# AVianEco/Softspoken

Hardware: AMD Instinct MI355X
Metric: audio-seconds processed/sec (whole node), 16 kHz mono (higher is better)
Workload: dtype f16x2

## Files before the change

softspoken_amd/csrc/conv4.hip:

```cpp
#include "kernels.h"
#include <cstdio>
#include <cstdlib>
#include <type_traits>
#include <utility>

namespace ss {

#ifdef SS_DEVBUILD
static int dev_env(const char* name, int dflt) { const char* v = getenv(name); return v ? atoi(v) : dflt; }
#else
static constexpr int dev_env(const char*, int dflt) { return dflt; }
#endif

typedef float f32x16 __attribute__((ext_vector_type(16)));
typedef float f32x4 __attribute__((ext_vector_type(4)));
typedef float f32x2 __attribute__((ext_vector_type(2)));
typedef __bf16 bf16x8 __attribute__((ext_vector_type(8)));
typedef __bf16 bf16x2 __attribute__((ext_vector_type(2)));
typedef _Float16 f16x8 __attribute__((ext_vector_type(8)));
typedef _Float16 f16x2 __attribute__((ext_vector_type(2)));
typedef short s16x2 __attribute__((ext_vector_type(2)));
typedef uint32_t u32x4 __attribute__((ext_vector_type(4)));
typedef uint32_t u32x2 __attribute__((ext_vector_type(2)));

// ... 61 lines not shown
    constexpr int KC = 32;
    constexpr bool DUO = NH > 1;
    static_assert(!DUO || (NT == 1 && NW * NH == 16 && RP == 0 && !FIRST && !FLAT && !PF2), "DUO: the plain A / B launches");
    constexpr bool RING = DUO && !BRES;
    static_assert(!RING || (SPLIT && NH == 4), "RING: f16x2, four 4-wave tiles");
    static_assert(!SPLIT || !PF2, "SPLIT: single-stage prefetch");
    static_assert(!RANK1 || (SPLIT && !RES && !RADD), "RANK1: conv1_1.B in f16x2 mode");
    static_assert(!(FIRST && SPLIT) || RANK1, "FIRST in f16x2 mode: the block's residual is the fp32 rank-1 term");
    static_assert(!FLAT || (NT == 1 && NW == 8 && BRES && (RADD || RP) && !POOL && !FIRST), "FLAT: conv9_1.B");
    static_assert(!PF2 || (BRES && !FIRST), "two-stage prefetch: resident-weight launches");
    static_assert(RP == 0 || (!RES && !RADD && !FIRST), "RP: a B launch that computes the block's projection itself (no r tensor)");
    static_assert(!FIRST || (NT == 1 && BRES && !RES && !RADD), "FIRST: conv1_1.B, one 32 -> 32 chunk, rank-1 residual");
    constexpr int kTapBytes = 2 * NT * 1024;
    constexpr int TAPS = RES ? 10 : 9;
    constexpr int NTHR = 64 * NW;
    constexpr int TH = 2 * NW;
    constexpr int PR = TH + 2;
    constexpr int kA = PR * kRowPitch;
    constexpr int NPA = PR * kPatch * 4;
    constexpr int AIT = (NPA + NTHR - 1) / NTHR;
    constexpr int NPB = (SPLIT ? 2 : 1) * TAPS * kTapBytes / 16;
    constexpr int BIT = BRES ? 1 : (DUO ? (NPB / 2 + NTHR - 1) / NTHR : (NPB + NTHR - 1) / NTHR);
    static_assert(!(RES && (RADD || POOL)), "RES is the A launch; RADD / POOL belong to B launches");
    static_assert(AIT <= 4, "edge flags are packed 8 bits per piece");
    extern __shared__ __attribute__((aligned(16))) char smem[];

    const int half = DUO ? __builtin_amdgcn_readfirstlane((int)threadIdx.x / NTHR) : 0;
    const int tid = DUO ? (int)threadIdx.x % NTHR : (int)threadIdx.x, lane = tid & 63;
    const int wave = __builtin_amdgcn_readfirstlane(tid >> 6);
    const int hh = lane >> 5, m = lane & 31;
    const int py = (m >> 1) & 1, px = (m & 1) | ((m >> 2) << 1);
    char* sA = smem + half * kA;
    const int sb_bytes = RING ? 2 * lds_b_bytes : lds_b_bytes;
    char* sB = smem + NH * kA;
    const int proj_steps = RP ? (a.C0x + a.C1x) / 16 : 0;
    constexpr bool proj_lds = RP > 0 && (BRES || NT == 3 || SPLIT);
    const char* sProj = smem + NH * kA + sb_bytes;
    const int proj_tiles = SPLIT ? a.Cout / 32 : NT;
    const int proj_bank = proj_steps * proj_tiles * 1024;
    const float* sBias = (const float*)(sProj + (proj_lds ? (SPLIT ? 2 : 1) * proj_bank : 0));
    constexpr int FW = 20, FROWS = PR + 3;
    float* sFb = (float*)sBias + 32;
    float* sF = sFb + 32;
    float* sFlat = (float*)sBias + 32;

    const int H = a.H, W = a.W, Cout = a.Cout;
    const int ngroups = Cout / (32 * NT);
    const int nch_r = (a.C0 + a.C1) / KC;
    const int nch = SPLIT ? 2 * nch_r : nch_r;
    const int all_taps = nch_r * TAPS;

    const int xcd = blockIdx.x & 7, local = (int)(blockIdx.x >> 3) * NH + half, gper = (int)(gridDim.x >> 3) * NH;
    const int per = (total_tiles + 7) >> 3;
    auto tile_of = [&](int loc, int it) -> int {
        if constexpr (RING) {
            const int total_pos = total_tiles / ngroups, per_pos = (total_pos + 7) >> 3;
            const int idx = loc + (it / ngroups) * gper;
            const int pos = xcd * per_pos + idx;
            return (idx < per_pos && pos < total_pos) ? pos * ngroups + it % ngroups : -1;
        }
        const int idx = loc + it * gper;
        const int t = xcd * per + idx;
        return (idx < per && t < total_tiles) ? t : -1;
    };
    auto tile_at = [&](int it) -> int { return tile_of(local, it); };
    struct Tile { int n, y0, x0, g; };
    auto decode = [&](int t) -> Tile {
        Tile d;
        d.g = t % ngroups; t /= ngroups;
        d.x0 = (t % a.tiles_x) * 16; t /= a.tiles_x;
        d.y0 = (t % a.tiles_y) * TH;
        d.n = t / a.tiles_y;
        return d;
    };

    uint32_t pix_full[AIT], pix_half[AIT], lds_off[AIT], flags = 0;
    const uint32_t part16 = (tid & 3) * 16;
    {
        const int Wh = W >> 1;
#pragma unroll
        for (int it = 0; it < AIT; ++it) {
            const int p = tid + NTHR * it;
            const int pix = p >> 2;
            const int pyy = pix / kPatch, pxx = pix - pyy * kPatch;
            lds_off[it] = pyy * kRowPitch + pxx * kPixPitch + part16;
            pix_full[it] = pyy * W + pxx;
            pix_half[it] = ((pyy + 1) >> 1) * Wh + ((pxx + 1) >> 1);
            const uint32_t f = (pyy == 0 ? 1u : 0u) | (pyy == PR - 1 ? 2u : 0u) | (pxx == 0 ? 4u : 0u) | (pxx == kPatch - 1 ? 8u : 0u) |
                               (p >= NPA ? 16u : 0u);
            flags |= f << (8 * it);
        }
    }
    u32x4 ra0[AIT], ra1[AIT];
    u32x4 rb[BIT];
    float rf = 0.f;
    static_assert(!FIRST || (PR + 2) * FW <= NTHR, "one feature value per thread");

    auto issue_patch = [&](const Tile& d, int ci, u32x4 (&ra)[AIT]) {
        if constexpr (FIRST) {
            if constexpr (SPLIT) { if (ci & 1) return; }
            const int fy = tid / FW, fx = tid - fy * FW;
            const int Y = d.y0 - 2 + fy, X = d.x0 - 2 + fx;
            rf = (tid < (PR + 2) * FW && (unsigned)Y < (unsigned)H && (unsigned)X < (unsigned)W)
                     ? a.rank1_src[((size_t)d.n * H + Y) * W + X] : 0.f;
            return;
        }
        const int ch = (SPLIT ? ci >> 1 : ci) * KC;
        const int64_t plane = (SPLIT && !(ci & 1)) ? a.lo_delta : 0;
        const char* base; uint32_t cs2, toff; bool up;
        if (ch < a.C0) {
            base = (const char*)a.src0 - kHdr + plane; cs2 = 2u * a.C0; up = false;
            toff = kHdr + ((((uint32_t)d.n * H + d.y0 - 1) * W + d.x0 - 1) * a.C0 + ch) * 2u;
        } else {
            base = (const char*)a.src1 - kHdr + plane; cs2 = 2u * a.C1; up = true;
            toff = kHdr + ((((uint32_t)d.n * (H >> 1) + (d.y0 >> 1) - 1) * (W >> 1) + (d.x0 >> 1) - 1) * a.C1 + (ch - a.C0)) * 2u;
        }
        uint32_t tm = (d.y0 == 0 ? 1u : 0u) | (d.y0 + TH == H ? 2u : 0u) | (d.x0 == 0 ? 4u : 0u) | (d.x0 + 16 == W ? 8u : 0u) | 16u;
        const uint32_t tp = toff + part16;
#pragma unroll
        for (int it = 0; it < AIT; ++it) {
            const uint32_t pix = up ? pix_half[it] : pix_full[it];
            uint32_t off = __umul24(pix, cs2) + tp;
            if (flags & (tm << (8 * it))) off = 0;
            ra[it] = *(const u32x4*)(base + off);
        }
    };
    auto issue_weights = [&](const Tile& d, int ci) {
        if constexpr (!BRES && !RING) {
            if constexpr (SPLIT) { if (ci & 1) return; }
            const char* wsrc = SPLIT ? (const char*)a.wpk + ((size_t)d.g * nch_r + (ci >> 1)) * 2 * (TAPS * kTapBytes)
                                     : (const char*)a.wpk + ((size_t)d.g * all_taps + ci * TAPS) * kTapBytes;
#pragma unroll
            for (int it = 0; it < BIT; ++it) {
                const int p = tid + NTHR * it;
                u32x4 v = {0u, 0u, 0u, 0u};
                if (p < NPB) v = *(const u32x4*)(wsrc + p * 16);
                rb[it] = v;
            }
        }
    };
    auto commit = [&](u32x4 (&ra)[AIT], bool patch, bool bank) {
        if constexpr (FIRST) return;
        if (patch) {
#pragma unroll
            for (int it = 0; it < AIT; ++it) {
                if ((it + 1) * NTHR <= NPA || !(flags & (16u << (8 * it)))) *(u32x4*)(sA + lds_off[it]) = ra[it];
            }
        }
        if constexpr (!BRES && !RING) {
            if (bank) {
#pragma unroll
                for (int it = 0; it < BIT; ++it) {
                    const int p = tid + NTHR * it;
                    if (p < NPB) *(u32x4*)(sB + p * 16) = rb[it];
                }
            }
        }
    };
    constexpr int NPH = NPB / 2;
    auto ring_duty = [&](int s, int n_chunks) {
        if constexpr (RING) {
            if (half > 1) return;
            const int k = (s >> 1) + 1;
            if (k >= n_chunks) return;
            if (!(s & 1)) {
                const char* wsrc = (const char*)a.wpk + ((size_t)(k % (ngroups * nch_r)) * 2 + half) * (TAPS * kTapBytes);
#pragma unroll
                for (int it = 0; it < BIT; ++it) {
                    const int p = tid + NTHR * it;
                    u32x4 v = {0u, 0u, 0u, 0u};
                    if (p < NPH) v = *(const u32x4*)(wsrc + p * 16);
                    rb[it] = v;
                }
            } else {
                char* dst = sB + (k & 1) * lds_b_bytes + half * (TAPS * kTapBytes);
#pragma unroll
                for (int it = 0; it < BIT; ++it) {
                    const int p = tid + NTHR * it;
                    if (p < NPH) *(u32x4*)(dst + p * 16) = rb[it];
                }
            }
        }
    };

    constexpr int RPH = RP >= 2 ? RP / 2 : RP;
    u32x4 pxh[(SPLIT && RP) ? RPH : 1], pxl[(SPLIT && RP) ? RPH : 1];
    auto issue_proj = [&](const Tile& d, int chunk, auto k0c, auto k1c) {
        constexpr int K0 = decltype(k0c)::value, K1 = decltype(k1c)::value;
        if constexpr (SPLIT && RP > 0 && K1 > K0) {
            const uint32_t t_full = kHdr + ((((uint32_t)d.n * H + d.y0 + 2 * wave) * W + d.x0) * a.C0x) * 2u;
            const uint32_t t_half = kHdr + ((((uint32_t)d.n * (H >> 1) + (d.y0 >> 1) + wave) * (W >> 1) + (d.x0 >> 1)) * a.C1x) * 2u;
            uint32_t zl = 0;
            asm volatile("" : "+v"(zl));
            const uint32_t xf_o = (uint32_t)((py * W + px) * a.C0x + hh * 8) * 2u + zl, xh_o = (uint32_t)((px >> 1) * a.C1x + hh * 8) * 2u + zl;
#pragma unroll
            for (int k = K0; k < K1; ++k) {
                const int sidx = chunk * RP + k, ch = sidx * 16;
                const char* base; uint32_t off;
                if (sidx >= proj_steps) { base = (const char*)a.xp0 - kHdr; off = 0; }
                else if (ch < a.C0x) { base = (const char*)a.xp0 - kHdr; off = t_full + xf_o + ch * 2u; }
                else { base = (const char*)a.xp1 - kHdr; off = t_half + xh_o + (ch - a.C0x) * 2u; }
                pxh[k - K0] = *(const u32x4*)(base + off);
                pxl[k - K0] = *(const u32x4*)(base + a.lo_delta + off);
            }
        }
    };

    int it_tile = 0;
    struct Stage { int ci; Tile d; };
    auto next_stage = [&](const Stage& s0, Stage& n) -> bool {
        n = s0; n.ci = s0.ci + 1;
        if (n.ci == nch) {
            n.ci = 0;
            const int t = tile_at(++it_tile);
            if (t < 0) return false;
            n.d = decode(t);
        }
        return true;
    };
    int my_stages = 0, max_stages = 0;
    if constexpr (DUO) {
        const int l0 = (int)(blockIdx.x >> 3) * NH;
        int n0 = 0, nmine = 0;
        while (tile_of(l0, n0) >= 0) ++n0;
        while (tile_of(l0 + half, nmine) >= 0) ++nmine;
        my_stages = nmine * nch;
        max_stages = n0 * nch;
        if (max_stages == 0) return;
    } else {
        if (tile_at(0) < 0) return;
    }
    Stage cs{0, decode((DUO && my_stages == 0) ? 0 : tile_at(0))}, n1 = cs, n2 = cs;

    if constexpr (BRES || RING) {
        const char* wsrc = (const char*)a.wpk;
        for (int p = tid; p < lds_b_bytes / 16; p += NTHR) *(u32x4*)(sB + p * 16) = *(const u32x4*)(wsrc + (size_t)p * 16);
    }
    for (int i = tid; i < Cout * (RES ? 2 : 1); i += NTHR)
        ((float*)sBias)[i] = i < Cout ? a.bias[i] : a.res_bias[i - Cout];
    if constexpr (proj_lds)
        for (int p = tid; p < (SPLIT ? 2 : 1) * proj_steps * proj_tiles * 64; p += NTHR) *(u32x4*)((char*)sProj + p * 16) = *(const u32x4*)((const char*)a.proj_w + (size_t)p * 16);
    u32x4 wfirst = {0u, 0u, 0u, 0u}, wr1 = {0u, 0u, 0u, 0u}, wfirst_lo = {0u, 0u, 0u, 0u};
    constexpr int NMT = (PR * kPatch + 31) / 32;
    int pf_off[2], pa_off[2]; uint32_t pflags = 0;
    if constexpr (FIRST) {
        for (int i = tid; i < 32; i += NTHR) sFb[i] = a.first_b[i];
        for (int i = tid; i < FROWS * FW; i += NTHR) sF[i] = 0.f;
        const float* w9 = a.first_w;
        auto wv = [&](int t) { return w9[t * 32 + m]; };
        if constexpr (SPLIT) {
            auto hi2 = [&](float x, float y) { return pack_f16(x, y); };
            auto lo2 = [&](float x, float y) { const f32x2 b = unpack_f16(pack_f16(x, y)); return pack_f16(x - b[0], y - b[1]); };
            if (hh == 0) {
                wfirst = u32x4{hi2(wv(0), wv(1)), hi2(wv(2), 0.f), hi2(wv(3), wv(4)), hi2(wv(5), 0.f)};
                wfirst_lo = u32x4{lo2(wv(0), wv(1)), lo2(wv(2), 0.f), lo2(wv(3), wv(4)), lo2(wv(5), 0.f)};
            } else {
                wfirst = u32x4{hi2(wv(6), wv(7)), hi2(wv(8), 0.f), 0u, 0u};
                wfirst_lo = u32x4{lo2(wv(6), wv(7)), lo2(wv(8), 0.f), 0u, 0u};
            }
        } else if (hh == 0) {
            wfirst = u32x4{pack_bf16(wv(0), wv(1)), pack_bf16(wv(2), 0.f), pack_bf16(wv(3), wv(4)), pack_bf16(wv(5), 0.f)};
            const float w = a.rank1_w[m];
            const float whi = (float)(__bf16)w, wlo = w - whi;
            wr1 = u32x4{pack_bf16(whi, whi), pack_bf16(wlo, 0.f), 0u, 0u};
        } else {
            wfirst = u32x4{pack_bf16(wv(6), wv(7)), pack_bf16(wv(8), 0.f), 0u, 0u};
        }
#pragma unroll
        for (int t = 0; t < 2; ++t) {
            const int q = 32 * (wave + NW * t) + m;
            const bool in = q < PR * kPatch;
            const int qq = in ? q : 0;
            const int qy = qq / kPatch, qx = qq - qy * kPatch;
            pf_off[t] = (qy + 2 * hh) * FW + qx;
            pa_off[t] = qy * kRowPitch + qx * kPixPitch + hh * 16;
            const uint32_t f = (qy == 0 ? 1u : 0u) | (qy == PR - 1 ? 2u : 0u) | (qx == 0 ? 4u : 0u) | (qx == kPatch - 1 ? 8u : 0u) | (in ? 0u : 16u);
            pflags |= f << (8 * t);
        }
    }
    u32x4 hk_lo[(FIRST && SPLIT) ? 2 : 1], hk_hi[(FIRST && SPLIT) ? 2 : 1];
    auto produce = [&](const Tile& d, int part) {
        const uint32_t tm = (d.y0 == 0 ? 1u : 0u) | (d.y0 + TH == H ? 2u : 0u) | (d.x0 == 0 ? 4u : 0u) | (d.x0 + 16 == W ? 8u : 0u) | 16u;
#pragma unroll
        for (int t = 0; t < 2; ++t) {
            if (wave + NW * t < NMT) {
                if constexpr (SPLIT) {
                    if (part) {
                        if (!(pflags & (16u << (8 * t)))) {
// ... 889 lines not shown
```

softspoken_amd/csrc/conv4_ups.hip:

```cpp
#include "kernels.h"
#include <cstdlib>
#include <type_traits>

namespace ss {

namespace {

typedef float f32x16 __attribute__((ext_vector_type(16)));
typedef float f32x4 __attribute__((ext_vector_type(4)));
typedef float f32x2 __attribute__((ext_vector_type(2)));
typedef _Float16 f16x8 __attribute__((ext_vector_type(8)));
typedef _Float16 f16x2 __attribute__((ext_vector_type(2)));
typedef uint32_t u32x4 __attribute__((ext_vector_type(4)));
typedef uint32_t u32x2 __attribute__((ext_vector_type(2)));

constexpr int kHdr = 256;
constexpr int kPix = 80;
constexpr int kRowR = 1472;
constexpr int kOdd = 720;
constexpr int kRowU = 896;
constexpr int kLowPlane = 6 * kRowU;
constexpr int kPatchBytes = 10 * kRowR;
constexpr int kBankR = 9 * 2048, kBankU = 16 * 2048;
constexpr int NW = 4, NH = 4, NTHR = 64 * NW;
// ... 295 lines not shown
    for (int i = half; i < NH - 1; ++i) lds_barrier();
}

namespace {
constexpr int kEntR = 10 * 2048;
constexpr int kEntRH = kEntR + 256;
constexpr int kEntU = 17 * 2048;
constexpr int kSlot = kEntU;
constexpr int kGL = (kEntU / 32 + NTHR - 1) / NTHR;
}

__global__ __launch_bounds__(NTHR * NH) __attribute__((amdgpu_waves_per_eu(4)))
void conv3x3_upsr_kernel(ConvArgs a, int total_tiles, int) {
    extern __shared__ __attribute__((aligned(16))) char smem[];
#ifdef SS_DEVBUILD
#define SS_ABL(bit) (a.dbg & (1 << (bit)))
#else
#define SS_ABL(bit) false
#endif
    const int half = __builtin_amdgcn_readfirstlane((int)threadIdx.x / NTHR);
    const int tid = (int)threadIdx.x % NTHR, lane = tid & 63;
    const int wave = __builtin_amdgcn_readfirstlane(tid >> 6);
    const int hh = lane >> 5, m = lane & 31;
    const int ca = wave & 1, cb = wave >> 1;
    const int X = m & 7, Y = m >> 3;
    char* sA = smem + half * kPatchBytes;
    char* sR = smem + NH * kPatchBytes;

    const int H = a.H, W = a.W, Cout = a.Cout;
    const int ngroups = Cout / 32;
    const int nreg = a.C0 / 32, nups = a.C1 / 32;
    const int nst = 3 * nreg + 2 * nups;
    const int group_bytes = nreg * (kEntRH + kEntR) + nups * 2 * kEntU;

    struct Sp { int sec, chunk, part; };
    auto sp_next = [&](Sp& p) -> bool {
        if (++p.part == (p.sec ? 2 : 3)) {
            p.part = 0;
            if (++p.chunk == (p.sec ? nups : nreg)) {
                p.chunk = 0; p.sec ^= 1;
                if (p.sec && nups == 0) p.sec = 0;
                return p.sec == 0;
            }
        }
        return false;
    };
    auto starts_entry = [&](const Sp& p) -> bool { return p.sec || p.part != 1; };
    auto needs_patch = [&](const Sp& p) -> bool { return p.sec ? p.part == 0 : p.part != 2; };
    auto entry_off = [&](const Sp& p) -> int {
        return p.sec ? nreg * (kEntRH + kEntR) + (2 * p.chunk + p.part) * kEntU : p.chunk * (kEntRH + kEntR) + (p.part == 2 ? kEntRH : 0);
    };
    auto entry_size = [&](const Sp& p) -> int { return p.sec ? kEntU : (p.part == 2 ? kEntR : kEntRH); };

    const int xcd = blockIdx.x & 7, local = (int)(blockIdx.x >> 3) * NH + half, gper = (int)(gridDim.x >> 3) * NH;
    const int total_pos = total_tiles / ngroups, per_pos = (total_pos + 7) >> 3;
    const int lim = min(per_pos, total_pos - xcd * per_pos);
    auto count_pos = [&](int loc) -> int { return lim > loc ? (lim - loc + gper - 1) / gper : 0; };
    struct Tile { int n, y0, x0, g; };
    auto decode_pos = [&](int pos, int g) -> Tile {
        Tile d;
        d.g = g;
        d.x0 = (pos % a.tiles_x) * 16; pos /= a.tiles_x;
        d.y0 = (pos % a.tiles_y) * 8;
        d.n = pos / a.tiles_y;
        return d;
    };
    const int my_pos = count_pos(local);
    const int my_stages = my_pos * ngroups * nst;
    const int max_stages = count_pos((int)(blockIdx.x >> 3) * NH) * ngroups * nst;
    if (max_stages == 0) return;

    constexpr int AIT = 3;
    uint32_t pix_full[AIT], lds_off[AIT], flags = 0;
    const uint32_t part16 = (tid & 3) * 16;
#pragma unroll
    for (int it = 0; it < AIT; ++it) {
        const int p = tid + NTHR * it, pix = p >> 2;
        const int pyy = pix / 18, pxx = pix - pyy * 18;
        lds_off[it] = pyy * kRowR + (pxx & 1) * kOdd + (pxx >> 1) * kPix + part16;
        pix_full[it] = pyy * W + pxx;
        const uint32_t f = (pyy == 0 ? 1u : 0u) | (pyy == 9 ? 2u : 0u) | (pxx == 0 ? 4u : 0u) | (pxx == 17 ? 8u : 0u) | (p >= 720 ? 16u : 0u);
        flags |= f << (8 * it);
    }
    uint32_t pix_low, lds_low, flags_low;
    {
        const int pix = tid >> 2;
        const int ly = pix / 10, lx = pix - ly * 10;
        lds_low = ly * kRowU + lx * kPix + part16;
        pix_low = ly * (W >> 1) + lx;
        flags_low = (ly == 0 ? 1u : 0u) | (ly == 5 ? 2u : 0u) | (lx == 0 ? 4u : 0u) | (lx == 9 ? 8u : 0u) | (tid >= 240 ? 16u : 0u);
    }
    u32x4 ra[AIT];
    auto issue_patch = [&](const Tile& d, const Sp& p) {
        if (SS_ABL(18)) return;
        const uint32_t tm = (d.y0 == 0 ? 1u : 0u) | (d.y0 + 8 == H ? 2u : 0u) | (d.x0 == 0 ? 4u : 0u) | (d.x0 + 16 == W ? 8u : 0u) | 16u;
        if (p.sec == 0) {
            const int64_t plane = p.part ? 0 : a.lo_delta;
            const char* base = (const char*)a.src0 - kHdr + plane;
            const uint32_t cs2 = 2u * a.C0;
            const uint32_t tp = kHdr + ((((uint32_t)d.n * H + d.y0 - 1) * W + d.x0 - 1) * a.C0 + p.chunk * 32) * 2u + part16;
#pragma unroll
            for (int it = 0; it < AIT; ++it) {
                uint32_t off = __umul24(pix_full[it], cs2) + tp;
                if (flags & (tm << (8 * it))) off = 0;
                ra[it] = *(const u32x4*)(base + off);
            }
        } else {
            const char* base = (const char*)a.src1 - kHdr;
            const uint32_t cs2 = 2u * a.C1;
            const uint32_t tp = kHdr + ((((uint32_t)d.n * (H >> 1) + (d.y0 >> 1) - 1) * (W >> 1) + (d.x0 >> 1) - 1) * a.C1 + p.chunk * 32) * 2u + part16;
            uint32_t off = __umul24(pix_low, cs2) + tp;
            if (flags_low & tm) off = 0;
            ra[0] = *(const u32x4*)(base + off);
            ra[1] = *(const u32x4*)(base + (off ? a.lo_delta + off : 0));
        }
    };
    auto commit = [&](int sec) {
        if (sec == 0) {
#pragma unroll
            for (int it = 0; it < AIT; ++it)
                if (!(flags & (16u << (8 * it)))) *(u32x4*)(sA + lds_off[it]) = ra[it];
        } else if (!(flags_low & 16u)) {
            *(u32x4*)(sA + lds_low) = ra[0];
            *(u32x4*)(sA + kLowPlane + lds_low) = ra[1];
        }
    };

    const int pos0 = xcd * per_pos + local;
    Tile cur = decode_pos(my_pos ? pos0 : 0, 0), nxt = cur;
    int cur_g = 0, cur_j = 0, nxt_g = 0, nxt_j = 0;
    bool nxt_ok = false;
    auto compute_next = [&]() {
        nxt_g = cur_g + 1; nxt_j = cur_j;
        if (nxt_g == ngroups) { nxt_g = 0; ++nxt_j; }
        nxt_ok = nxt_j < my_pos;
        if (nxt_ok) nxt = decode_pos(pos0 + nxt_j * gper, nxt_g);
    };
    struct Cur { Sp sp; Tile d; bool ok; };
    auto advance = [&](Cur& c) {
        if (sp_next(c.sp)) { c.d = nxt; c.ok = nxt_ok; }
    };
    Cur ip{Sp{0, 0, 0}, cur, true};

    {
        Sp p{0, 0, 0};
        for (int e = 0; e < 3; ++e) {
            const char* src = (const char*)a.wpk + entry_off(p);
            const int np = entry_size(p) / 16;
            for (int q = (int)threadIdx.x; q < np; q += NTHR * NH) *(u32x4*)(sR + e * kSlot + q * 16) = *(const u32x4*)(src + (size_t)q * 16);
            do sp_next(p); while (!starts_entry(p));
        }
    }
    Sp rq{0, 0, 0};
    int rq_g = 0, rq_t = 0, rq_e = 0, rq_slot = 0;
    auto rq_advance = [&]() {
        if (starts_entry(rq)) { ++rq_e; rq_slot = rq_slot == 2 ? 0 : rq_slot + 1; }
        ++rq_t;
        if (sp_next(rq)) { if (++rq_g == ngroups) rq_g = 0; }
    };
    if (half & 1) for (int i = 0; i < (half == 1 ? 2 : 3); ++i) rq_advance();
    auto ring_issue = [&]() {
        if (!(half & 1)) return;
        if (!SS_ABL(19) && rq_t < max_stages && rq_e >= 3 && starts_entry(rq)) {
            const int total = entry_size(rq) / 16;
            const int h0 = ((total / 2 + 63) / 64) * 64;
            const int base = half == 1 ? 0 : h0, cnt = half == 1 ? h0 : total - h0;
            const char* src = (const char*)a.wpk + (size_t)rq_g * group_bytes + entry_off(rq) + base * 16;
            char* dst = sR + rq_slot * kSlot + base * 16 + wave * 1024;
#pragma unroll
            for (int it = 0; it < kGL; ++it) {
                const int idx = tid + NTHR * it;
                if (idx < cnt)
                    __builtin_amdgcn_global_load_lds((const __attribute__((address_space(1))) void*)(src + (size_t)idx * 16),
                                                     (__attribute__((address_space(3))) void*)(uintptr_t)(dst + it * NTHR * 16), 16, 0, 0);
            }
        }
        rq_advance();
    };

    issue_patch(ip.d, ip.sp);
    commit(0);
    if (my_stages == 0) ip.ok = false;
    else do advance(ip); while (ip.ok && !needs_patch(ip.sp));
    if (ip.ok) issue_patch(ip.d, ip.sp);
    __syncthreads();

    f32x16 acc, racc;
    auto mm = [&](const u32x4& w, const u32x4& x, const f32x16& c) -> f32x16 { return SS_ABL(16) ? c : mfma(w, x, c); };
    const int base_r = 2 * Y * kRowR + X * kPix + hh * 16;
    const int base_u = Y * kRowU + X * kPix + hh * 16;
    const int boff0 = lane * 16;
    const uint32_t st_off = (uint32_t)(((2 * Y + ca) * W + 2 * X + cb) * Cout + hh * 8) * 2u;
    const uint32_t r_lane = (uint32_t)(32 * hh + 4 * X + 2 * ca + cb) * 32u;
    int tap_r[9];
#pragma unroll
    for (int t = 0; t < 9; ++t) {
        const int dy = t / 3, dx = t % 3;
        tap_r[t] = (ca + dy) * kRowR + ((cb + dx) & 1) * kOdd + ((cb + dx) >> 1) * kPix;
    }
    int tap_u[4];
#pragma unroll
    for (int t = 0; t < 4; ++t) tap_u[t] = (ca + (t >> 1)) * kRowU + (cb + (t & 1)) * kPix;
    constexpr int kCentreU = kRowU + kPix;

    int jit_n = 0;
#ifdef SS_DEVBUILD
    uint32_t st_prev = 0, st_sub = 0, st_sum[9] = {0u, 0u, 0u, 0u, 0u, 0u, 0u, 0u, 0u};
#endif
    auto substamp = [&](int seg) {
#ifdef SS_DEVBUILD
        if (a.stamps) { const uint32_t t = (uint32_t)__builtin_amdgcn_s_memtime(); if (seg >= 5) st_sum[seg] += t - st_sub; st_sub = t; }
// ... 108 lines not shown
#pragma unroll
            for (int sub = 0; sub < 2; ++sub) {
                const u32x4 w = *(const u32x4*)(ent + boff0 + 16 * 2048 + sub * 1024);
                const u32x4 xh = *(const u32x4*)(sA + base_u + kCentreU + sub * 32), xl = *(const u32x4*)(sA + kLowPlane + base_u + kCentreU + sub * 32);
                racc = mm(w, xl, racc);
                racc = mm(w, xh, racc);
            }
        } else {
            const char* bb = ent + boff0 + wave * 4 * 2048;
            constexpr int PM = 3;
            u32x4 ph[PM], wf[PM];
            auto load2 = [&](int st, int slot) {
                if (SS_ABL(17)) return;
                const int tap = st >> 1, sub = st & 1;
                ph[slot] = *(const u32x4*)(sA + base_u + tap_u[tap] + sub * 32);
                wf[slot] = *(const u32x4*)(bb + tap * 2048 + sub * 1024);
            };
#pragma unroll
            for (int st = 0; st < PM - 1; ++st) load2(st, st);
#pragma unroll
            for (int st = 0; st < 8; ++st) {
                if (st + PM - 1 < 8) load2(st + PM - 1, (st + PM - 1) % PM);
                acc = mm(wf[st % PM], ph[st % PM], acc);
            }
#pragma unroll
            for (int sub = 0; sub < 2; ++sub) {
                const u32x4 w = *(const u32x4*)(ent + boff0 + 16 * 2048 + sub * 1024);
                const u32x4 xh = *(const u32x4*)(sA + base_u + kCentreU + sub * 32);
                racc = mm(w, xh, racc);
            }
        }
        if (a.dbg & 32) __builtin_amdgcn_s_setprio(0);
        jitter(1);
        vm_lds_barrier();
        jitter(2);
        const bool more = stage_no + 1 < my_stages;
        constexpr bool next_has_patch = KIND == 0 || KIND == 2 || KIND == 4;
        const int next_sec = KIND == 0 ? 0 : KIND == 2 ? ((c == nreg - 1 && nups) ? 1 : 0) : (c == nups - 1 ? 0 : 1);
        const bool np = next_has_patch && more;
        substamp(0);
        if (np) commit(next_sec);
        substamp(5);
        if (last && !SS_ABL(20)) {
            char* rq_p = (char*)a.res_out +
                         ((((((uint32_t)cur.n * (H >> 1) + (cur.y0 >> 1) + Y) * (W >> 4) + (cur.x0 >> 4)) * (uint32_t)ngroups) + cur.g) * 2048u + r_lane);
            *(f32x4*)(rq_p) = f32x4{racc[0], racc[1], racc[2], racc[3]};
            *(f32x4*)(rq_p + 16) = f32x4{racc[4], racc[5], racc[6], racc[7]};
            *(f32x4*)(rq_p + a.lo_delta) = f32x4{racc[8], racc[9], racc[10], racc[11]};
            *(f32x4*)(rq_p + a.lo_delta + 16) = f32x4{racc[12], racc[13], racc[14], racc[15]};
        }
        if (last) { acc_done = acc; done_off = (((uint32_t)cur.n * H + cur.y0) * W + cur.x0) * Cout + cur.g * 32; have_done = true; }
        if (KIND == 1 && c == 0 && have_done && !SS_ABL(20)) { store_h(); have_done = false; }
        if (KIND == 1 && c == 0) compute_next();
        if (last && more) { cur = nxt; cur_g = nxt_g; cur_j = nxt_j; }
        substamp(6);
        if (np) {
            do advance(ip); while (ip.ok && !needs_patch(ip.sp));
            if (ip.ok) issue_patch(ip.d, ip.sp);
        }
        substamp(7);
        ring_issue();
        substamp(8);
        jitter(3);
        lds_barrier();
        jitter(4);
        if (KIND != 0) e_slot = e_slot == 2 ? 0 : e_slot + 1;
        ++stage_no;
    };
    using K0 = std::integral_constant<int, 0>; using K1 = std::integral_constant<int, 1>; using K2 = std::integral_constant<int, 2>;
    using K3 = std::integral_constant<int, 3>; using K4 = std::integral_constant<int, 4>;
    const int my_pg = my_pos * ngroups, max_pg = max_stages / nst;
    for (int i = 0; i < half; ++i) lds_barrier();
    for (int pg = 0; pg < max_pg; ++pg) {
        if (pg < my_pg) {
            for (int c = 0; c < nreg; ++c) { stage(K0{}, c); stage(K1{}, c); stage(K2{}, c); }
            for (int c = 0; c < nups; ++c) { stage(K3{}, c); stage(K4{}, c); }
        } else {
            for (int st = 0; st < nst; ++st) { vm_lds_barrier(); ring_issue(); lds_barrier(); }
        }
    }
    for (int i = half; i < NH - 1; ++i) lds_barrier();
    if (have_done && !SS_ABL(20)) store_h();
#ifdef SS_DEVBUILD
    if (a.stamps && lane == 0) {
        uint32_t* sp = (uint32_t*)a.stamps + (((size_t)blockIdx.x * NH + half) * NW + wave) * 16;
        for (int i = 0; i < 5; ++i) sp[i] = st_sum[i];
        sp[5] = (uint32_t)jit_n; sp[6] = st_sum[5]; sp[7] = st_sum[6]; sp[8] = st_sum[7]; sp[9] = st_sum[8];
    }
#endif
#undef SS_ABL
}

namespace {

struct UpsChoice { bool ok; int total, lds_b, grid; size_t lds; };

UpsChoice choose_ups(ConvArgs& a, int num_cus) {
    UpsChoice c{};
    static const int on = dev_env("SOFTSPOKEN_UPS", 1);
    if (!on) return c;
    if (!a.plain || !a.src0 || !a.src1 || !a.out || !a.wpk || !a.bias || !a.range_flag || a.lo_delta <= 0) return c;
    if (a.res_out || a.res_in || a.pool_out || a.rank1_src || a.first_w || a.flat_part || a.proj_w || !a.relu || a.R0 || a.R1) return c;
    if (a.Cout != 32 || a.C0 < 32 || a.C1 < 32 || a.C0 % 32 || a.C1 % 32 || a.H % 8 || a.W % 16 || ((a.H | a.W) & 1)) return c;
    if ((double)a.N * a.H * a.W * std::max(a.Cout, std::max(a.C0, a.C1)) * 2.0 + kHdr >= 4294967296.0) return c;
    a.tiles_y = a.H / 8; a.tiles_x = a.W / 16;
    const long total_l = (long)a.N * a.tiles_y * a.tiles_x;
    if (total_l <= 0 || total_l > 0x7fffffff) return c;
    c.total = (int)total_l;
    c.lds_b = (a.C0 / 32) * 2 * kBankR + (a.C1 / 32) * 2 * kBankU;
    c.lds = (size_t)NH * kPatchBytes + c.lds_b + (size_t)a.Cout * 4;
    if (c.lds > 160 * 1024) return c;
    c.grid = (num_cus + 7) / 8 * 8;
    if (c.grid * NH > c.total) c.grid = ((c.total + NH - 1) / NH + 7) / 8 * 8;
    c.ok = true;
    return c;
}

}

namespace {

struct UpsrChoice { bool ok; int total, grid; size_t lds; };

UpsrChoice choose_upsr(ConvArgs& a, int num_cus) {
// ... 65 lines not shown
```

softspoken_amd/csrc/engine.hip:

```cpp
#include "engine.h"

#include <algorithm>
#include <chrono>
#include <cmath>
#include <cstdio>
#include <cstdlib>
#include <cstring>

namespace ss {

static thread_local std::string g_err;

int fail(ss_ctx* c, int code, const std::string& msg) {
    g_err = msg;
    if (c) c->err = msg;
    return code;
}
const char* thread_error() { return g_err.c_str(); }

#ifdef SS_DEVBUILD
int dev_env(const char* name, int dflt) { const char* v = getenv(name); return v ? atoi(v) : dflt; }
#endif

double now_ms() { return std::chrono::duration<double, std::milli>(std::chrono::steady_clock::now().time_since_epoch()).count(); }
// ... 71 lines not shown
    for (const WsTensor& t : kWsTensors) {
        offs.push_back(total + kActHeader);
        total += kActHeader + (((size_t)n * t.H * t.W * t.C * es + 255) & ~(size_t)255);
    }
    const int planes = c->prec == kF16x2 ? 2 : 1;
    const size_t feat_b = (size_t)n * 128 * 256 * 4, flat_b = (size_t)n * 64 * 4 * 256 * 4;
    hipError_t e = ws_malloc(c, &w.arena, total * planes);
    if (e != hipSuccess) { what = "activation workspace (" + std::to_string(total * planes >> 20) + " MiB)"; free_ws(w); return e; }
    if ((e = ws_malloc(c, (void**)&w.feat, feat_b)) != hipSuccess || (e = ws_malloc(c, (void**)&w.flat, flat_b)) != hipSuccess) {
        what = "activation workspace"; free_ws(w); return e;
    }
    for (int pl = 0; pl < planes; ++pl)
        for (size_t off : offs) {
            e = hipMemsetAsync((char*)w.arena + pl * total + off - kActHeader, 0, kActHeader, stream);
            if (e != hipSuccess) { what = "hipMemsetAsync"; free_ws(w); return e; }
        }
    for (size_t i = 0; i < offs.size(); ++i) w.act[kWsTensors[i].n] = (char*)w.arena + offs[i];
    w.lo_delta = planes == 2 ? (int64_t)total : 0;
    w.bytes = (int64_t)(total * planes + feat_b + flat_b);
    w.chunk = n;
    return hipSuccess;
}

int ensure_workspace(ss_ctx* c, int n) {
    if (n <= c->ws[0].chunk) return SS_OK;
    HIPCHK(c, hipStreamSynchronize(c->stream));
    if (c->lane_stream) HIPCHK(c, hipStreamSynchronize(c->lane_stream));
    free_workspace(c);
    std::string what;
    const hipError_t e = alloc_ws(c, n, c->stream, c->ws[0], what);
    if (e != hipSuccess) return fail(c, what == "hipMemsetAsync" ? SS_ERR_HIP : SS_ERR_NOMEM, what + ": " + hipGetErrorString(e));
    return SS_OK;
}

static bool ensure_lane(ss_ctx* c, int n) {
    Workspace& w = c->ws[1];
    if (w.chunk >= n) return true;
    if (!c->lane_stream) {
        if (hipStreamCreateWithFlags(&c->lane_stream, hipStreamNonBlocking) != hipSuccess) { c->lane_stream = nullptr; return false; }
        if (hipEventCreateWithFlags(&c->lane_ev_in, hipEventDisableTiming) != hipSuccess || hipEventCreateWithFlags(&c->lane_ev_out, hipEventDisableTiming) != hipSuccess) return false;
    }
    hipStreamSynchronize(c->lane_stream);
    free_ws(w);
    size_t free_b = 0, total_b = 0;
    if (hipMemGetInfo(&free_b, &total_b) != hipSuccess || (int64_t)free_b < c->ws[0].bytes + ((int64_t)4 << 30)) return false;
    std::string what;
    if (alloc_ws(c, n, c->lane_stream, w, what) != hipSuccess) { (void)hipGetLastError(); return false; }
    return true;
}

struct ConvExtra { const float* first_w = nullptr; const float* first_b = nullptr; const void* flat_w = nullptr; const void* flat_w4 = nullptr; float* flat_part = nullptr; int store_out = 1; };

static int base_dbg() {
    return (dev_env("SOFTSPOKEN_PRIO", 1) ? 32 : 0) | dev_env("SOFTSPOKEN_DBG", 0);
}

#ifdef SS_DEVBUILD
struct StageStamps {
    void* d_st = nullptr;
    static constexpr size_t st_bytes = (size_t)4096 * 8 * 16 * 4;
    int begin(ss_ctx* c, hipStream_t stream, const std::string& name, ConvArgs& a) {
        const char* want = getenv("SOFTSPOKEN_STAMP_LAYER");
        if (want && name == want) { HIPCHK(c, hipMalloc(&d_st, st_bytes)); HIPCHK(c, hipMemsetAsync(d_st, 0, st_bytes, stream)); a.stamps = d_st; }
        return SS_OK;
    }
    int end(ss_ctx* c, hipStream_t stream, const std::string& name, int n) {
        if (!d_st) return SS_OK;
        std::vector<uint32_t> h(st_bytes / 4);
        HIPCHK(c, hipMemcpyAsync(h.data(), d_st, st_bytes, hipMemcpyDeviceToHost, stream));
        HIPCHK(c, hipStreamSynchronize(stream));
        double sum[12] = {0, 0, 0, 0, 0, 0, 0, 0, 0, 0, 0, 0}, stages = 0; int waves = 0;
        for (size_t w = 0; w < h.size() / 16; ++w) if (h[w * 16 + 5]) {
            ++waves; stages += h[w * 16 + 5];
            for (int i = 0; i < 5; ++i) sum[i] += h[w * 16 + i];
            for (int i = 5; i < 12; ++i) sum[i] += h[w * 16 + i + 1];
        }
        if (waves)
            fprintf(stderr, "[stamps] %s n=%d: %d waves, %.1f stages/wave; cycles per stage: mfma %.0f | barrier1 %.0f | commit+issue %.0f (wait for loads %.0f, LDS writes %.0f, next stage %.0f, patch loads %.0f, one stamp %.0f) | barrier2 %.0f | epilogue %.0f (f16x2: residual add incl. its wait %.0f, the last stage's work %.0f)\n",
                    name.c_str(), n, waves, stages / waves, sum[0] / stages, sum[1] / stages, sum[2] / stages, sum[5] / stages, sum[6] / stages, sum[7] / stages, sum[8] / stages, sum[9] / stages, sum[3] / stages, sum[4] / stages, sum[10] / stages, sum[11] / stages);
        hipFree(d_st); d_st = nullptr;
        return SS_OK;
    }
};
#else
struct StageStamps {
    int begin(ss_ctx*, hipStream_t, const std::string&, ConvArgs&) { return SS_OK; }
    int end(ss_ctx*, hipStream_t, const std::string&, int) { return SS_OK; }
};
#endif

template <typename Launch>
static int conv_launch(ss_ctx* c, hipStream_t stream, const char* variant, const std::string& layer, ConvArgs& a, double flops, double bytes,
                       double issued, Launch&& launch) {
    StageStamps stamps;
    if (int rc = stamps.begin(c, stream, layer, a)) return rc;
    {
        ScopedLaunch sl(c, stream, std::string(variant) + "/" + layer, flops, bytes, issued);
        HIPCHK(c, launch(a));
    }
    return stamps.end(c, stream, layer, a.N);
}

static void mark_written(ss_ctx* c, const Workspace& ws, const void* p) {
#ifdef SS_DEVBUILD
    if (!p) return;
    for (const auto& kv : ws.act)
        if (kv.second == p) { c->dbg_written.insert(kv.first); return; }
// ... 490 lines not shown
```

softspoken_amd/csrc/kernels.h:

```cpp
#pragma once
#include <hip/hip_runtime.h>
#include <stdint.h>
#include <atomic>

namespace ss {

inline hipError_t allow_full_lds(const void* kernel, std::atomic<uint64_t>& done) {
    int dev = 0;
    hipError_t e = hipGetDevice(&dev);
    if (e != hipSuccess) return e;
    const uint64_t bit = 1ull << (dev & 63);
    if (done.load(std::memory_order_acquire) & bit) return hipSuccess;
    e = hipFuncSetAttribute(kernel, hipFuncAttributeMaxDynamicSharedMemorySize, 160 * 1024);
    if (e == hipSuccess) done.fetch_or(bit, std::memory_order_release);
    return e;
}

struct ConvArgs {
    const void* src0; const void* src1;
    const void* res0; const void* res1;
    const void* wpk;
    const float* bias;
    const float* rank1_src;
    const float* rank1_w;
    void* out;
    void* pool_out;
    int N, H, W, C0, C1, R0, R1, Cout;
    int relu;
    int tiles_y, tiles_x;
    int dbg;
    const float* first_w; const float* first_b;
    const void* flat_w; float* flat_part;
    int store_out;
    const void* flat_w4;
    void* res_out; const float* res_bias;
    const void* res_in;
    const void* wpk_b; const float* bias_a;
    int plain;
    const void* proj_w;
    const void* xp0; const void* xp1; int C0x, C1x;
    int64_t lo_delta;
    int* range_flag;
    void* stamps;
};
hipError_t launch_conv3x3_v2(const ConvArgs& a, bool bf16, int NT, int num_cus, hipStream_t s);
const char* conv_v2_variant(const ConvArgs& a, bool bf16, int NT, int num_cus);
int conv_v2_flat_groups(bool bf16);
bool conv_v4_supports(const ConvArgs& a, int NT, int num_cus, int prec);
const char* conv_v4_variant(const ConvArgs& a, int NT, int num_cus, int prec);
int conv_v4_flat_groups();
hipError_t launch_conv3x3_v4(const ConvArgs& a, int NT, int num_cus, int prec, hipStream_t s);

bool conv_ups_supports(const ConvArgs& a, int num_cus);
const char* conv_ups_variant();
size_t conv_ups_weight_bytes(int C0, int C1);
hipError_t launch_conv3x3_ups(const ConvArgs& a, int num_cus, hipStream_t s);
bool conv_upsr_supports(const ConvArgs& a, int num_cus);
const char* conv_upsr_variant();
size_t conv_upsr_weight_bytes(int C0, int C1, int Cout);
hipError_t launch_conv3x3_upsr(const ConvArgs& a, int num_cus, hipStream_t s);

bool conv_ups32_supports(const ConvArgs& a, int NT, int MTW, int num_cus);
const char* conv_ups32_variant(int NT, int MTW);
size_t conv_ups32_weight_bytes(int C0, int C1, int Cout);
hipError_t launch_conv3x3_ups32(const ConvArgs& a, int NT, int MTW, int num_cus, hipStream_t s);

bool conv1_stream_supports(const ConvArgs& a);
const char* conv1_stream_variant(const ConvArgs& a, int form);
size_t conv1_stream_weight_bytes();
hipError_t launch_conv1_stream(const ConvArgs& a, int form, int rows_per_unit, int num_cus, hipStream_t s);

struct Head1dWeights { float w1[4][4][3], b1[4], w2[4][4][3], wr[4][4], b2r[4], wo[4], bo, fscale; };
hipError_t launch_mask_head_parts(const float* parts, int n_parts, const float* flat_bias, const Head1dWeights& hw, float* logits,
                                  int N, hipStream_t s);
hipError_t launch_spec_tail(const void* x, int64_t lo_delta, const float* w , const float* bias, float* spec, int N, int prec,
                            hipStream_t s);

static constexpr int kMelLo = 10, kMelHi = 32, kMelPitch = 43;
struct FrontendTables {
    const float4* pretw;
    const float2* w2048;
    const int* mel_start;
    const int* mel_count;
    const int* mel_off;
    const float* mel_w;
    int mel_nw;
    const float* mel_wp;
    int dbg;
    const float2* win2;
    const float2* twt;
    const float2* wkt;
    const float* mel_wq;
    const int* mel_p0;
};
static constexpr int kMelPairsLo = 9, kMelPairsHi = 20, kMelRow = 60;
static constexpr int kPwWords = 816;
hipError_t launch_frontend(const float* arena, const int64_t* win_off, int n, const FrontendTables& t, float* feat,
// ... 38 lines not shown
```

Baseline: 30530.

## Interleave ring conv work items across output-channel groups side by side

Adds a 'side-by-side' ordering for the ring-scheduled conv kernels. Each workgroup now starts at a different output-channel group (wg % ngroups) and strides by the grid size over a flattened (position, group) space, rather than every workgroup walking all groups of one position in sequence. The weight ring preload and the refill addressing are adjusted to match the starting group and step. The intent is to balance work across workgroups and spread concurrent weight-bank reads across groups, at the cost of less reuse of input patches across the groups of one position.

Result: faster. 30840, median of 6 (+1.0%).

```diff
diff --git a/softspoken_amd/csrc/conv4.hip b/softspoken_amd/csrc/conv4.hip
--- a/softspoken_amd/csrc/conv4.hip
+++ b/softspoken_amd/csrc/conv4.hip
@@ -137,12 +137,15 @@
 
     const int xcd = blockIdx.x & 7, local = (int)(blockIdx.x >> 3) * NH + half, gper = (int)(gridDim.x >> 3) * NH;
     const int per = (total_tiles + 7) >> 3;
+#ifdef SS_DEVBUILD
+    const bool order_seq = !(a.dbg & 512);
+#else
+    constexpr bool order_seq = !kOrderSideBySide;
+#endif
     auto tile_of = [&](int loc, int it) -> int {
         if constexpr (RING) {
-            const int total_pos = total_tiles / ngroups, per_pos = (total_pos + 7) >> 3;
-            const int idx = loc + (it / ngroups) * gper;
-            const int pos = xcd * per_pos + idx;
-            return (idx < per_pos && pos < total_pos) ? pos * ngroups + it % ngroups : -1;
+            const RingItem r = ring_item(xcd, loc / NH, (int)(gridDim.x >> 3), it, loc % NH, total_tiles / ngroups, ngroups, order_seq);
+            return r.pos >= 0 ? r.pos * ngroups + r.g : -1;
         }
         const int idx = loc + it * gper;
         const int t = xcd * per + idx;
@@ -243,13 +246,17 @@
         }
     };
     constexpr int NPH = NPB / 2;
+    const int ring_g0 = RING ? ring_group0((int)(blockIdx.x >> 3), ngroups, order_seq) : 0;
+    const int ring_gstep = RING ? ring_group_step((int)(gridDim.x >> 3), ngroups, order_seq) : 0;
+    int ring_g = ring_g0, ring_c = 0;
     auto ring_duty = [&](int s, int n_chunks) {
         if constexpr (RING) {
             if (half > 1) return;
             const int k = (s >> 1) + 1;
             if (k >= n_chunks) return;
             if (!(s & 1)) {
-                const char* wsrc = (const char*)a.wpk + ((size_t)(k % (ngroups * nch_r)) * 2 + half) * (TAPS * kTapBytes);
+                if (++ring_c == nch_r) { ring_c = 0; ring_g += ring_gstep; if (ring_g >= ngroups) ring_g -= ngroups; }
+                const char* wsrc = (const char*)a.wpk + ((size_t)(ring_g * nch_r + ring_c) * 2 + half) * (TAPS * kTapBytes);
 #pragma unroll
                 for (int it = 0; it < BIT; ++it) {
                     const int p = tid + NTHR * it;
@@ -318,7 +325,7 @@
     Stage cs{0, decode((DUO && my_stages == 0) ? 0 : tile_at(0))}, n1 = cs, n2 = cs;
 
     if constexpr (BRES || RING) {
-        const char* wsrc = (const char*)a.wpk;
+        const char* wsrc = (const char*)a.wpk + (RING ? (size_t)ring_g0 * nch_r * 2 * (TAPS * kTapBytes) : 0);
         for (int p = tid; p < lds_b_bytes / 16; p += NTHR) *(u32x4*)(sB + p * 16) = *(const u32x4*)(wsrc + (size_t)p * 16);
     }
     for (int i = tid; i < Cout * (RES ? 2 : 1); i += NTHR)
diff --git a/softspoken_amd/csrc/conv4_ups.hip b/softspoken_amd/csrc/conv4_ups.hip
--- a/softspoken_amd/csrc/conv4_ups.hip
+++ b/softspoken_amd/csrc/conv4_ups.hip
@@ -371,10 +371,14 @@
     };
     auto entry_size = [&](const Sp& p) -> int { return p.sec ? kEntU : (p.part == 2 ? kEntR : kEntRH); };
 
-    const int xcd = blockIdx.x & 7, local = (int)(blockIdx.x >> 3) * NH + half, gper = (int)(gridDim.x >> 3) * NH;
-    const int total_pos = total_tiles / ngroups, per_pos = (total_pos + 7) >> 3;
-    const int lim = min(per_pos, total_pos - xcd * per_pos);
-    auto count_pos = [&](int loc) -> int { return lim > loc ? (lim - loc + gper - 1) / gper : 0; };
+#ifdef SS_DEVBUILD
+    const bool order_seq = !(a.dbg & 512);
+#else
+    constexpr bool order_seq = !kOrderSideBySide;
+#endif
+    const int xcd = blockIdx.x & 7, wg = (int)(blockIdx.x >> 3), nwg = (int)(gridDim.x >> 3);
+    const int total_pos = total_tiles / ngroups;
+    const int g0 = ring_group0(wg, ngroups, order_seq), gstep = ring_group_step(nwg, ngroups, order_seq);
     struct Tile { int n, y0, x0, g; };
     auto decode_pos = [&](int pos, int g) -> Tile {
         Tile d;
@@ -384,9 +388,9 @@
         d.n = pos / a.tiles_y;
         return d;
     };
-    const int my_pos = count_pos(local);
-    const int my_stages = my_pos * ngroups * nst;
-    const int max_stages = count_pos((int)(blockIdx.x >> 3) * NH) * ngroups * nst;
+    const int my_items = ring_items(xcd, wg, nwg, half, total_pos, ngroups, order_seq);
+    const int my_stages = my_items * nst;
+    const int max_stages = ring_items(xcd, wg, nwg, 0, total_pos, ngroups, order_seq) * nst;
     if (max_stages == 0) return;
 
     constexpr int AIT = 3;
@@ -445,15 +449,13 @@
         }
     };
 
-    const int pos0 = xcd * per_pos + local;
-    Tile cur = decode_pos(my_pos ? pos0 : 0, 0), nxt = cur;
-    int cur_g = 0, cur_j = 0, nxt_g = 0, nxt_j = 0;
+    Tile cur = decode_pos(my_items ? ring_item(xcd, wg, nwg, 0, half, total_pos, ngroups, order_seq).pos : 0, g0), nxt = cur;
+    int cur_i = 0, nxt_i = 0;
     bool nxt_ok = false;
     auto compute_next = [&]() {
-        nxt_g = cur_g + 1; nxt_j = cur_j;
-        if (nxt_g == ngroups) { nxt_g = 0; ++nxt_j; }
-        nxt_ok = nxt_j < my_pos;
-        if (nxt_ok) nxt = decode_pos(pos0 + nxt_j * gper, nxt_g);
+        nxt_i = cur_i + 1;
+        nxt_ok = nxt_i < my_items;
+        if (nxt_ok) { const RingItem r = ring_item(xcd, wg, nwg, nxt_i, half, total_pos, ngroups, order_seq); nxt = decode_pos(r.pos, r.g); }
     };
     struct Cur { Sp sp; Tile d; bool ok; };
     auto advance = [&](Cur& c) {
@@ -464,18 +466,18 @@
     {
         Sp p{0, 0, 0};
         for (int e = 0; e < 3; ++e) {
-            const char* src = (const char*)a.wpk + entry_off(p);
+            const char* src = (const char*)a.wpk + (size_t)g0 * group_bytes + entry_off(p);
             const int np = entry_size(p) / 16;
             for (int q = (int)threadIdx.x; q < np; q += NTHR * NH) *(u32x4*)(sR + e * kSlot + q * 16) = *(const u32x4*)(src + (size_t)q * 16);
             do sp_next(p); while (!starts_entry(p));
         }
     }
     Sp rq{0, 0, 0};
-    int rq_g = 0, rq_t = 0, rq_e = 0, rq_slot = 0;
+    int rq_g = g0, rq_t = 0, rq_e = 0, rq_slot = 0;
     auto rq_advance = [&]() {
         if (starts_entry(rq)) { ++rq_e; rq_slot = rq_slot == 2 ? 0 : rq_slot + 1; }
         ++rq_t;
-        if (sp_next(rq)) { if (++rq_g == ngroups) rq_g = 0; }
+        if (sp_next(rq)) { rq_g += gstep; if (rq_g >= ngroups) rq_g -= ngroups; }
     };
     if (half & 1) for (int i = 0; i < (half == 1 ? 2 : 3); ++i) rq_advance();
     auto ring_issue = [&]() {
@@ -690,7 +692,7 @@
         if (last) { acc_done = acc; done_off = (((uint32_t)cur.n * H + cur.y0) * W + cur.x0) * Cout + cur.g * 32; have_done = true; }
         if (KIND == 1 && c == 0 && have_done && !SS_ABL(20)) { store_h(); have_done = false; }
         if (KIND == 1 && c == 0) compute_next();
-        if (last && more) { cur = nxt; cur_g = nxt_g; cur_j = nxt_j; }
+        if (last && more) { cur = nxt; cur_i = nxt_i; }
         substamp(6);
         if (np) {
             do advance(ip); while (ip.ok && !needs_patch(ip.sp));
@@ -707,7 +709,7 @@
     };
     using K0 = std::integral_constant<int, 0>; using K1 = std::integral_constant<int, 1>; using K2 = std::integral_constant<int, 2>;
     using K3 = std::integral_constant<int, 3>; using K4 = std::integral_constant<int, 4>;
-    const int my_pg = my_pos * ngroups, max_pg = max_stages / nst;
+    const int my_pg = my_items, max_pg = max_stages / nst;
     for (int i = 0; i < half; ++i) lds_barrier();
     for (int pg = 0; pg < max_pg; ++pg) {
         if (pg < my_pg) {
diff --git a/softspoken_amd/csrc/engine.hip b/softspoken_amd/csrc/engine.hip
--- a/softspoken_amd/csrc/engine.hip
+++ b/softspoken_amd/csrc/engine.hip
@@ -147,7 +147,7 @@
 struct ConvExtra { const float* first_w = nullptr; const float* first_b = nullptr; const void* flat_w = nullptr; const void* flat_w4 = nullptr; float* flat_part = nullptr; int store_out = 1; };
 
 static int base_dbg() {
-    return (dev_env("SOFTSPOKEN_PRIO", 1) ? 32 : 0) | dev_env("SOFTSPOKEN_DBG", 0);
+    return (dev_env("SOFTSPOKEN_PRIO", 1) ? 32 : 0) | (dev_env("SOFTSPOKEN_ORDER", kOrderSideBySide ? 1 : 0) ? 512 : 0) | dev_env("SOFTSPOKEN_DBG", 0);
 }
 
 #ifdef SS_DEVBUILD
diff --git a/softspoken_amd/csrc/kernels.h b/softspoken_amd/csrc/kernels.h
--- a/softspoken_amd/csrc/kernels.h
+++ b/softspoken_amd/csrc/kernels.h
@@ -43,6 +43,30 @@
     int* range_flag;
     void* stamps;
 };
+static constexpr bool kOrderSideBySide = true;
+struct RingItem { int pos, g; };
+__host__ __device__ inline int ring_lim(int xcd, int total_pos) {
+    const int per_pos = (total_pos + 7) >> 3, left = total_pos - xcd * per_pos;
+    return left < 0 ? 0 : left < per_pos ? left : per_pos;
+}
+__host__ __device__ inline int ring_group0(int wg, int ngroups, bool seq) { return seq ? 0 : wg % ngroups; }
+__host__ __device__ inline int ring_group_step(int G, int ngroups, bool seq) { return seq ? 1 % ngroups : G % ngroups; }
+__host__ __device__ inline RingItem ring_item(int xcd, int wg, int G, int item, int tile, int total_pos, int ngroups, bool seq) {
+    const int lim = ring_lim(xcd, total_pos);
+    int quad, g;
+    if (seq) { quad = wg + (item / ngroups) * G; g = item % ngroups; }
+    else { const int j = wg + item * G; quad = j / ngroups; g = j - quad * ngroups; }
+    const int idx = 4 * quad + tile;
+    return RingItem{idx < lim ? xcd * ((total_pos + 7) >> 3) + idx : -1, g};
+}
+__host__ __device__ inline int ring_items(int xcd, int wg, int G, int tile, int total_pos, int ngroups, bool seq) {
+    const int lim = ring_lim(xcd, total_pos);
+    const int quads = lim > tile ? (lim - tile + 3) >> 2 : 0;
+    if (seq) return quads > wg ? (quads - wg + G - 1) / G * ngroups : 0;
+    const int n = quads * ngroups;
+    return n > wg ? (n - wg + G - 1) / G : 0;
+}
+
 hipError_t launch_conv3x3_v2(const ConvArgs& a, bool bf16, int NT, int num_cus, hipStream_t s);
 const char* conv_v2_variant(const ConvArgs& a, bool bf16, int NT, int num_cus);
 int conv_v2_flat_groups(bool bf16);
```
